# abhro/MonteCarloScattering.jl

Hardware: AMD Instinct MI355X
Metric: particle-scatter steps/sec + wall-time per iter, 10^6 particles, 1->8 MI355X (higher is better)
Workload: dtype f64

## Files before the change

montecarloscattering.jl_amd/csrc/mcs_transport.hip:

```cpp
#include "mcs_device.h"
#define MCS_DEVICE_FAST_SQRT 1
#include "../../include/mcs_math.h"
#include "../../include/mcs_math_f32.h"

#pragma clang fp contract(off)

#ifndef MCS_WAVES_PER_SIMD
#define MCS_WAVES_PER_SIMD 2
#endif
#ifndef MCS_REFILL_MIN
#define MCS_REFILL_MIN 12
#endif
#ifndef MCS_DEFER_K
#define MCS_DEFER_K 8
#endif
#ifndef MCS_PASSES_PER_ITER
#define MCS_PASSES_PER_ITER 6
#endif
#ifndef MCS_MERGE_POLL_MASK
#define MCS_MERGE_POLL_MASK 15u
#endif
#ifndef MCS_TAIL_CROSS
#define MCS_TAIL_CROSS 1
#endif
#ifdef MCS_INLINE_COLD
#define MCS_COLD __forceinline__
#else
#define MCS_COLD __noinline__
#endif

typedef const __attribute__((address_space(4))) KArgs CK;

namespace {

#define PI_ MCS_SC(3.141592653589793)
#define TWOPI_ MCS_SC(6.283185307179586)
#define HALFPI_ MCS_SC(1.5707963267948966)
#define SIN_UL MCS_SC(0x1.fffffffffffffp-1)
#define MP_ MCS_SC(MCS_MP)
#define CC_ MCS_SC(MCS_C)

__device__ __forceinline__ double rcp_refined(double b) {
  double r = __builtin_amdgcn_rcp(b);
// ... 1323 lines not shown
    else if (j == 6) off = a->L.energy_esc_feb + ion + (long long)a->P.n_ions * iter;
    if (v != 0.0) gadd_f64(&a->T[off], v);
  }
  for (int i = threadIdx.x; i < ng; i += blockDim.x) {
    const double v0 = S_fl[i], v1 = S_fl[MCS_MAXNE + i], v2 = S_fl[2 * MCS_MAXNE + i];
    if (v0 != 0.0) gadd_f64(&a->T[a->L.pxx_flux + i], v0);
    if (v1 != 0.0) gadd_f64(&a->T[a->L.pxz_flux + i], v1);
    if (v2 != 0.0) gadd_f64(&a->T[a->L.energy_flux + i], v2);
    const int c = S_nc[i];
    if (c) gadd_u64(&a->I[MCS_I_NUM_CROSSINGS + i], (unsigned long long)c);
  }
  for (int i = threadIdx.x; i < MCS_NA_C; i += blockDim.x) {
    const double w = S_wc[i];
    if (w != 0.0) gadd_f64(&a->T[a->L.weight_coupled + i + (long long)MCS_NA_C * (a->i_ion - 1)], w);
  }
  for (int i = threadIdx.x; i <= MCS_PSD_MAX; i += blockDim.x) {
    const long long o = i + (long long)(MCS_PSD_MAX + 1) * (a->i_ion - 1);
    const double e = S_eff[0][i], w = S_eff[1][i];
    if (e != 0.0) gadd_f64(&a->T[a->L.esc_energy_eff + o], e);
    if (w != 0.0) gadd_f64(&a->T[a->L.esc_num_eff + o], w);
  }
}

template <bool PLAIN, bool LOSSY = false, bool PLAIN_ETF = false, bool SLICED = false>
__device__ __forceinline__ void transport_body(const KArgs* __restrict__ ka) {
  CK* a = (CK*)ka;
  if (a->n_dev && *a->n_dev == 0) return;
  const int ne = a->P.n_grid + 2, ng = a->P.n_grid, ntc = a->tb.n_tcuts;
  block_prologue(a);
  __syncthreads();

  Hot h;
  h.m = vconst(a->m); h.x_grid_stop = vconst(a->P.x_grid_stop); h.xn_coarse = vconst(a->P.xn_per_coarse);
  h.u2 = sconst(a->P.u2); h.eta = sconst(a->P.eta_mfp); h.zzq = sconst(a->zzq); h.mc = sconst(a->mc);
  h.feb_down = sconst(a->P.feb_downstream); h.pcut = sconst(a->pcut); h.pmax_cutoff = sconst(a->pmax_cutoff);
  h.feb_up = sconst(a->P.feb_upstream); h.age_max = sconst(a->P.age_max); h.inj_frac = sconst(a->inj_frac);
  h.xn_fine = sconst(a->P.xn_per_fine); h.aa = sconst(a->aa);
  h.n_grid = sconsti(ng); h.i_grid_feb = sconsti(a->P.i_grid_feb); h.n_tcuts = sconsti(ntc); h.n_xspec = sconsti(a->tb.n_xspec);
  h.custom_epsB = a->P.use_custom_epsB != 0; h.etf = a->P.energy_transfer_frac > 0;
  h.dont_scatter = a->P.dont_scatter != 0; h.rad_losses = a->P.do_rad_losses != 0;
  h.do_tcuts = a->P.do_tcuts != 0; h.dont_DSA = a->P.dont_DSA != 0;
  {
    int ob = 0;
    for (int i = threadIdx.x; i < ne; i += blockDim.x) ob |= S_bsin[i] != 0.0;
    h.oblique = __builtin_amdgcn_readfirstlane(__syncthreads_or(ob)) != 0;
  }
  h.every_pass = h.custom_epsB || (h.rad_losses && h.aa < 1) || h.dont_scatter;
  h.odd_cfg = h.feb_down > 0 || h.dont_DSA || h.inj_frac < 1 || h.aa < 1 || h.n_xspec != 0;
  if (PLAIN) {
    h.custom_epsB = false; h.etf = PLAIN_ETF ? h.etf : false; h.dont_scatter = false; h.dont_DSA = false; h.oblique = false;
    h.every_pass = false; h.odd_cfg = false;
  }
  double l_bcmb = 0, l_pe_crit = 0, l_game_crit = 0;
  if (LOSSY) {
    h.every_pass = false; h.custom_epsB = false; h.dont_scatter = false; h.rad_losses = true;
    l_bcmb = sconst(a->P.B_CMBz); l_pe_crit = sconst(a->P.pe_crit); l_game_crit = sconst(a->P.game_crit);
  }

  mcsm::HotCoef kc;
  kc.S0 = vconst(MCS_SIN_0); kc.S1 = vconst(MCS_SIN_1); kc.S2 = vconst(MCS_SIN_2); kc.S3 = vconst(MCS_SIN_3);
  kc.S4 = vconst(MCS_SIN_4); kc.S5 = vconst(MCS_SIN_5);
  kc.C0 = vconst(MCS_COS_0); kc.C1 = vconst(MCS_COS_1); kc.C2 = vconst(MCS_COS_2); kc.C3 = vconst(MCS_COS_3);
  kc.C4 = vconst(MCS_COS_4); kc.C5 = vconst(MCS_COS_5);
  kc.A0 = vconst(MCS_ASIN_0); kc.A1 = vconst(MCS_ASIN_1); kc.A2 = vconst(MCS_ASIN_2); kc.A3 = vconst(MCS_ASIN_3);
  kc.A4 = vconst(MCS_ASIN_4); kc.A5 = vconst(MCS_ASIN_5); kc.A6 = vconst(MCS_ASIN_6); kc.A7 = vconst(MCS_ASIN_7);
  kc.A8 = vconst(MCS_ASIN_8); kc.A9 = vconst(MCS_ASIN_9); kc.A10 = vconst(MCS_ASIN_10); kc.A11 = vconst(MCS_ASIN_11);
  kc.A12 = vconst(MCS_ASIN_12);
  kc.R0 = vconst(MCS_TWO_OVER_PI); kc.R1 = vconst(MCS_PIO2_0); kc.R2 = vconst(MCS_PIO2_1); kc.R3 = vconst(MCS_PIO2_2);

  Pt p;
  Rng rng;
  p.weight = 0; p.ptot_pf = 1; p.pb_pf = 0; p.p_perp = 1; p.gam_pf = 1; p.x = 0; p.x_old = 0; p.phi = 0; p.prp = 0; p.acctime = 0;
  p.xn_per = 1; p.dphi = 0; p.gyro_denom = 0; p.gyro_rad = 0; p.gyro_rad_tot = 0; p.gyro_period = 0; p.t_step = 0;
  p.rp_val = 1; p.cm_val = 1; p.rg_val = 1; p.x_dt = 0; p.t_ev = 0; p.flags = 0; p.ovr_inc = 0; p.n_ovr = 0u;
  p.z_gsf = 1; p.z_bcos = 1; p.z_ux = 0; p.z_gef = 1; p.z_lo = 0; p.z_hi = 0; p.t_hi = 0; p.t_lo = 0; p.c_gef = 0; p.c_tev = 0;
  p.i_grid = 0; p.i_grid_old = 0; p.ig3 = 0; p.helix = 0; p.tcut = 1; p.n_retro = 0; p.downstream = false; p.inj = false;
  rng.init(0ull);
  int act = 0;
#define active (act != 0)
  bool exhausted = false;
  int evw = 0;
  double phi_prev = 0.0;
  long long k = -1;
  const unsigned lane = __lane_id();
  const unsigned long long n_resume = SLICED ? (unsigned long long)a->n_resume : 0ull;
  const long long fresh_lo = SLICED ? a->fresh_lo : 0ll;
  long long n_pop = a->n;
  if (a->n_dev) {
    const long long v = *a->n_dev;
    n_pop = (long long)(((unsigned long long)(unsigned)__builtin_amdgcn_readfirstlane((int)(v >> 32)) << 32) | (unsigned)__builtin_amdgcn_readfirstlane((int)v));
  }
  const unsigned long long n = n_resume + (unsigned long long)(n_pop - fresh_lo);
  const unsigned budget = SLICED ? (unsigned)__builtin_amdgcn_readfirstlane(a->budget_trips) : 0u;
  const int claim_max = SLICED ? __builtin_amdgcn_readfirstlane(a->claim_max) : 64;
  const unsigned long_draws = SLICED ? (unsigned)__builtin_amdgcn_readfirstlane((int)a->long_draws) : 0u;
  unsigned mtick_ex = 0;

  const unsigned wv = threadIdx.x >> 6;
  int mrole = 0;
  unsigned mtick = 0, mpoll_mask = ~0u;
  if (blockDim.x == 256u && a->tail_merge) {
    const unsigned s0 = S_msimd[0], s1 = S_msimd[1], s2 = S_msimd[2], s3 = S_msimd[3];
    const bool distinct = ((1u << s0) | (1u << s1) | (1u << s2) | (1u << s3)) == 15u;
    const unsigned slot = (unsigned)__builtin_amdgcn_s_getreg((3 << 11) | (0 << 6) | 4);
    if (__builtin_amdgcn_readfirstlane(distinct ? 1 : 0))
      mrole = __builtin_amdgcn_readfirstlane((int)(((S_msimd[wv] ^ slot) & 1u) == 0u ? 2 : 1));
  }
  auto pair_of = [&](unsigned& partner) -> unsigned {
    const unsigned mine = S_msimd[wv], want = mine ^ 1u;
    const unsigned pw = S_msimd[0] == want ? 0u : (S_msimd[1] == want ? 1u : (S_msimd[2] == want ? 2u : 3u));
    partner = (unsigned)__builtin_amdgcn_readfirstlane((int)pw);
    return (unsigned)__builtin_amdgcn_readfirstlane((int)(mine >> 1));
  };
#ifdef MCS_PROF
  const unsigned gw__ = (blockIdx.x * 4u + wv) & 8191u;
  if (lane == 0) { g_wave[gw__][0] = __builtin_amdgcn_s_memrealtime(); g_wave[gw__][1] = 0; }
  unsigned long long xp__ = 0, xr__ = 0, xl__ = 0, xf__ = 0;
#endif
  const bool waiting_on = __builtin_amdgcn_readfirstlane((int)(a->wait_full != 0 && blockDim.x == 256u)) != 0;
  const unsigned refill_min = claim_max < 64 ? (unsigned)(64 - claim_max + 1)
                                             : (unsigned)__builtin_amdgcn_readfirstlane(a->refill_min);
  unsigned refill_at = refill_min;
  unsigned ev_pending = 0;
  bool ring_on = false;
  unsigned rb = 0u - 256u;
  unsigned rrow = 0u;
  unsigned ringD = 1u;
  unsigned defer_k = h.every_pass ? 1u : (unsigned)__builtin_amdgcn_readfirstlane(a->defer_k);
  p.npush = 0;
  auto build_batch = [&](const unsigned long long am, const unsigned L) {
    const unsigned D = 64u / L;
    const unsigned M = 65536u / D + 1u;
    const unsigned rank = below(am);
    if (active) {
      S_evf[wv][3][128u + rank] = __hiloint2double((int)rng.k0, (int)rng.k1);
      S_evf[wv][4][128u + rank] = __hiloint2double((int)rng.n, 0);
      S_evf[wv][5][128u + rank] = 1 - p.cm_val;
    }
    const unsigned q = (lane * M) >> 16, jw = lane - q * D;
    const bool valid = q < L;
    const unsigned qq = valid ? q : 0u;
    const double w1 = S_evf[wv][3][128u + qq], w2 = S_evf[wv][4][128u + qq], womc = S_evf[wv][5][128u + qq];
    double eU1, es, ec, ecd, esd, essd;
    scatter_draws((uint32_t)__double2hiint(w1), (uint32_t)__double2loint(w1), ((uint32_t)__double2hiint(w2) >> 1) + jw, kc, eU1, es, ec);
    scatter_cone(eU1, es, womc, ecd, esd, essd);
    if (valid) {
      S_evf[wv][0][128u + lane] = ecd; S_evf[wv][1][128u + lane] = esd; S_evf[wv][2][128u + lane] = ec; S_evf[wv][6][128u + lane] = essd;
    }
    if (active) { rb = rng.n; rrow = rank * D; }
    ringD = D;
  };
  constexpr bool TAIL_LOOP = !LOSSY;
  const unsigned tail_loop_L = TAIL_LOOP ? (unsigned)__builtin_amdgcn_readfirstlane(a->tail_loop) : 0u;
  bool done = false;
  while (!done) {
    ev_pending += (unsigned)(__popcll(__builtin_amdgcn_ballot_w64(p.npush > 0)) + __popcll(__builtin_amdgcn_ballot_w64(p.npush > 1)));
    p.npush = 0;
    const unsigned long long act_mask = __builtin_amdgcn_ballot_w64(active);
    const int n_idle = 64 - __popcll(act_mask);
    unsigned Lh = 64u - (unsigned)n_idle;
    const bool waitl = (p.flags & F_WAIT) != 0;
    const unsigned n_wait = (unsigned)__popcll(__builtin_amdgcn_ballot_w64(waitl));
    ++mtick;
    if (MCS_UNLIKELY(((ev_pending >= 64u) | ((unsigned)n_idle + n_wait >= refill_at) | ((mtick & mpoll_mask) == 0u)) != 0)) {
      if (ev_pending >= 64u) { drain_events(a, wv, lane, false); ev_pending &= 63u; PROF_ADD(3, 1); }
      if (n_wait > 0u && (exhausted || (unsigned)n_idle + n_wait >= refill_min)) {
        if (waitl) p.flags = (p.flags & ~F_WAIT) | F_NOPARK;
        PROF_ADD(36, 1); PROF_ADD(37, n_wait);
      }
      const unsigned long long idle = ~__builtin_amdgcn_ballot_w64(active);
      if ((unsigned)n_idle + n_wait >= refill_min && !exhausted && idle != 0ull) {
        const int nfree = __popcll(idle);
        int nidle = nfree < claim_max - (64 - nfree) ? nfree : claim_max - (64 - nfree);
        nidle = nidle > 0 ? nidle : 0;
        const int leader = __ffsll((long long)idle) - 1;
        unsigned long long base = 0;
        if ((int)lane == leader) base = atomicAdd(a->work_counter, (unsigned long long)nidle);
        base = __shfl(base, leader);
        if (__builtin_amdgcn_readfirstlane(base >= n ? 1 : 0)) {
          exhausted = true;
          defer_k = 1u;
          ring_on = !LOSSY && __builtin_amdgcn_readfirstlane(a->tail_ring) != 0;
          mtick_ex = mtick;
          if (mrole != 0 || budget != 0u) mpoll_mask = MCS_MERGE_POLL_MASK;
#ifdef MCS_PROF_TAIL
          if (lane == 0) S_ttgate[wv] = 1u;
#endif
#ifdef MCS_PROF
          if (lane == 0 && g_wave[gw__][1] == 0) { g_wave[gw__][1] = __builtin_amdgcn_s_memrealtime(); g_wave[gw__][3] = (unsigned long long)__popcll(act_mask); }
#endif
        } else if (!active) {
          const int rank = (int)below(idle);
          const unsigned long long idx = base + (unsigned long long)rank;
          if (rank < nidle && idx >= n_resume && idx < n) {
            k = fresh_lo + (long long)(idx - n_resume);
            load_particle(a, h, k, p, rng);
            act = -1; evw = 0; rb = 0u - 256u;
            __builtin_amdgcn_s_waitcnt(0x0F70);
          }
        }
        if (SLICED && !exhausted && __builtin_amdgcn_readfirstlane(base < n_resume ? 1 : 0)) {
          drain_events(a, wv, lane, true); ev_pending = 0u;
          const unsigned long long left = n_resume - base;
          const unsigned cnt_r = (unsigned)(left < (unsigned long long)nidle ? left : (unsigned long long)nidle);
          const unsigned rank = below(idle);
          double* const box = &S_evf[wv][0][0];
          for (unsigned b0 = 0; b0 < cnt_r; b0 += MCS_MB_SLOTS) {
            const unsigned cb = cnt_r - b0 < MCS_MB_SLOTS ? cnt_r - b0 : MCS_MB_SLOTS;
            const double* src = a->strag_in + (base + b0) * MCS_STRAG_WORDS;
            for (unsigned i = lane; i < MCS_MB_WORDS * MCS_MB_SLOTS; i += 64u) {
              const unsigned j = i / MCS_MB_SLOTS, r = i % MCS_MB_SLOTS;
              if (r < cb) box[i] = src[r * MCS_STRAG_WORDS + j];
            }
            __builtin_amdgcn_fence(__ATOMIC_RELEASE, "wavefront"); __builtin_amdgcn_wave_barrier(); __builtin_amdgcn_fence(__ATOMIC_ACQUIRE, "wavefront");
            if (!active && rank >= b0 && rank < b0 + cb) {
              mb_load(wv, rank - b0, p, rng, k, evw, phi_prev);
              refresh_thr<LOSSY>(h, p);
              act = -1; rb = rng.n - 256u;
            }
            __builtin_amdgcn_fence(__ATOMIC_RELEASE, "wavefront"); __builtin_amdgcn_wave_barrier(); __builtin_amdgcn_fence(__ATOMIC_ACQUIRE, "wavefront");
          }
        }
        PROF_ADD(5, 1); PROF_ADD(6, nidle);
      }
      auto take_donation = [&](unsigned mpair, unsigned mpartner) {
        __builtin_amdgcn_fence(__ATOMIC_ACQUIRE, "workgroup");
        const unsigned cntm = (unsigned)__builtin_amdgcn_readfirstlane((int)S_mcount[mpair]);
        const unsigned long long idle_now = ~__builtin_amdgcn_ballot_w64(active);
        const unsigned r = below(idle_now);
        if (!active && r < cntm) {
          mb_load(mpartner, r, p, rng, k, evw, phi_prev);
          refresh_thr<LOSSY>(h, p);
          rb = rng.n - 256u;
          act = -1;
        }
        mrole = 0; mpoll_mask = budget != 0u ? MCS_MERGE_POLL_MASK : ~0u;
      };
      const bool closing = SLICED && budget != 0u && exhausted &&
                           (long_draws != 0u ? __builtin_amdgcn_ballot_w64(active && rng.n < long_draws) == 0ull : mtick - mtick_ex >= budget);
      if (mrole != 0 && exhausted) {
        unsigned mpartner;
        const unsigned mpair = pair_of(mpartner);
        const int nlive = __popcll(__builtin_amdgcn_ballot_w64(active));
        if (mrole == 2) {
          unsigned st = 0u;
          if (lane == 0) {
            S_mlive[wv] = (unsigned)nlive;
            st = (nlive == 0 || closing) ? atomicCAS(&S_mstate[mpair], 0u, 2u) : __hip_atomic_load(&S_mstate[mpair], __ATOMIC_RELAXED, __HIP_MEMORY_SCOPE_WORKGROUP);
          }
          st = (unsigned)__builtin_amdgcn_readfirstlane((int)st);
          if (st == 1u) {
            take_donation(mpair, mpartner);
            if (lane == 0) S_mstate[mpair] = 2u;
          } else if (st == 2u || nlive == 0 || closing) { mrole = 0; mpoll_mask = budget != 0u ? MCS_MERGE_POLL_MASK : ~0u; }
        } else {
          const int room = 64 - (int)__builtin_amdgcn_readfirstlane((int)S_mlive[mpartner]);
          if (nlive == 0 || closing) {
            if (lane == 0) (void)atomicCAS(&S_mstate[mpair], 0u, 2u);
            mrole = 0; mpoll_mask = budget != 0u ? MCS_MERGE_POLL_MASK : ~0u;
          } else if (nlive <= MCS_MB_SLOTS && nlive <= room) {
            drain_events(a, wv, lane, true); ev_pending = 0u;
            if (active) mb_store(wv, below(__builtin_amdgcn_ballot_w64(active)), p, rng, k, evw, phi_prev);
            rb = rng.n - 256u;
// ... 15 lines not shown
          const int nlive = __popcll(am_x);
          const int leader = __ffsll((long long)am_x) - 1;
          unsigned long long base = 0;
          if ((int)lane == leader) base = atomicAdd(a->strag_count, (unsigned long long)nlive);
          base = __shfl(base, leader);
          drain_events(a, wv, lane, true); ev_pending = 0u;
          const unsigned rank = below(am_x);
          double* const box = &S_evf[wv][0][0];
          for (unsigned b0 = 0; b0 < (unsigned)nlive; b0 += MCS_MB_SLOTS) {
            const unsigned cb = (unsigned)nlive - b0 < MCS_MB_SLOTS ? (unsigned)nlive - b0 : MCS_MB_SLOTS;
            if (active && rank >= b0 && rank < b0 + cb) mb_store(wv, rank - b0, p, rng, k, evw, phi_prev);
            __builtin_amdgcn_fence(__ATOMIC_RELEASE, "wavefront"); __builtin_amdgcn_wave_barrier(); __builtin_amdgcn_fence(__ATOMIC_ACQUIRE, "wavefront");
            double* dst = a->strag_out + (base + b0) * MCS_STRAG_WORDS;
            for (unsigned i = lane; i < MCS_MB_WORDS * MCS_MB_SLOTS; i += 64u) {
              const unsigned j = i / MCS_MB_SLOTS, r = i % MCS_MB_SLOTS;
              if (r < cb) dst[r * MCS_STRAG_WORDS + j] = box[i];
            }
            __builtin_amdgcn_fence(__ATOMIC_RELEASE, "wavefront"); __builtin_amdgcn_wave_barrier(); __builtin_amdgcn_fence(__ATOMIC_ACQUIRE, "wavefront");
          }
          act = 0; p.flags = 0; p.helix = 0; evw = 0;
        }
        mrole = 0;
      }
      if (exhausted) refill_at = 64u;
      const unsigned long long am_hk = __builtin_amdgcn_ballot_w64(active);
      Lh = (unsigned)__popcll(am_hk);
      done = (am_hk == 0ull) & exhausted;
    }
    {
      [[maybe_unused]] const int na__ = __popcll(__builtin_amdgcn_ballot_w64(active));
      PROF_ADD(0, 1); PROF_ADD(8, na__);
#ifdef MCS_PROF
      if (exhausted) { xp__ += 1; xl__ += (unsigned long long)na__; }
#endif
    }
    double t_clock = p.t_step;
    const int wi = (((evw & 3) | p.flags) | (h.every_pass ? 1 : 0)) & act;
    const bool waits = (p.flags & F_WAIT) != 0;
    const bool want = (wi != 0) & !waits;
    PROF_LANES(13, want);
#ifdef MCS_PROF_TAIL
    const bool rare_any__ = PROF_GATE && __builtin_amdgcn_ballot_w64(want) != 0ull;
    unsigned long long tt0__ = 0;
    if (rare_any__) tt0__ = __builtin_amdgcn_s_memtime();
#endif
    bool waits_now = false;
    bool loss_done = false;
    const unsigned long long m_want = __builtin_amdgcn_ballot_w64(want);
    const unsigned long long m_urgent = __builtin_amdgcn_ballot_w64(want & ((wi & F_NOPARK) != 0));
    const bool enter = (m_urgent != 0ull) | ((unsigned)__popcll(m_want) >= defer_k);
    if (MCS_UNLIKELY(want & enter)) {
      PROF_ADD(12, 1);
#ifdef MCS_PROF_TAIL
#define TT_MARK(slot) do { const unsigned long long tn__ = __builtin_amdgcn_s_memtime(); if (PROF_GATE && (threadIdx.x & 63u) == (unsigned)(__ffsll((long long)__ballot(1)) - 1)) atomicAdd(&S_prof[slot], tn__ - tm__); tm__ = __builtin_amdgcn_s_memtime(); } while (0)
      unsigned long long tm__ = __builtin_amdgcn_s_memtime();
#else
#define TT_MARK(slot) do { } while (0)
#endif
      const double cm_in = p.cm_val;
      const bool moved = (evw & 4) != 0, thr = (evw & 2) != 0;
      bool ev = (evw & 1) != 0, ev_x = false;
      bool up_due = false, xn_due = false, feb_due = false;
      if (__builtin_amdgcn_ballot_w64(thr) != 0ull) {
        const bool fwd = p.x > p.x_old;
        const bool same_zone = (fwd & (p.z_hi > p.x)) | (!fwd & (p.z_lo <= p.x));
        const bool ev_up = ((p.x >= h.x_grid_stop) & ((p.x_old < h.x_grid_stop) | ((p.x_old < p.prp) & (p.x >= p.prp)))) | (p.x > p.x_dt);
        const bool ev_xn = !LOSSY & ((p.x > p.gyro_rad_tot) != (p.xn_per == h.xn_coarse));
        ev_x = thr & !same_zone;
        up_due = thr & ev_up; xn_due = thr & ev_xn;
        feb_due = thr & (p.i_grid <= h.i_grid_feb) & p.inj & (p.x < h.feb_up);
        ev = ev | up_due | xn_due | feb_due;
      }
      [[maybe_unused]] const bool unusual = (p.flags != 0) | (p.helix >= MCS_HELIX_CAP) | h.every_pass;
      const bool post_pending = moved && (ev || ev_x || (p.flags & F_INJCHK) != 0);
      int end = -1;
      bool t_due = false, age_out = false;
      if (__builtin_amdgcn_ballot_w64(ev) != 0ull) {
        t_due = ev & p.downstream & (p.acctime >= p.t_ev);
        age_out = (h.age_max > 0) & (p.acctime > h.age_max);
      }
      const bool etf_due = h.etf & ev_x & !(p.inj | (p.downstream & (p.x < 0))) & (p.x_old <= 0);
      bool full = (p.flags & ~F_CM) != 0 || p.helix >= MCS_HELIX_CAP || h.every_pass || etf_due || h.custom_epsB ||
                  (ev && (h.odd_cfg || up_due || age_out || feb_due));
      TT_MARK(32);
      if (!full && ev_x) full = !plain_crossing(a, h, p, ev_pending);
      TT_MARK(33);
      if (waiting_on && !exhausted) {
        waits_now = full & moved & ((p.flags & F_NOPARK) == 0);
        p.flags = waits_now ? (p.flags | F_WAIT) : p.flags;
        full = full & !waits_now;
      }
      if (__builtin_amdgcn_ballot_w64(full || (!waits_now && ((p.flags & F_CM) != 0 || t_due || xn_due))) != 0ull) {
      if (!full && !waits_now) {
        if (p.flags & F_CM) {
          refresh_scatter(a, p, h.aa, h.aa * MP_ * CC_, h.eta);
          p.flags = 0;
        }
        if (t_due) {
          if (h.do_tcuts && !(p.tcut > h.n_tcuts) && p.acctime >= tcut_next_of(a, h, p.tcut)) {
            tcut_track(a, p.tcut, p.weight, p.ptot_pf);
            p.tcut += 1;
          }
          refresh_time(a, h, p);
        }
        if (xn_due) {
          p.xn_per = p.x > p.gyro_rad_tot ? h.xn_coarse : h.xn_fine;
          p.flags |= F_CM;
          refresh_move(a, h, p);
        }
      }
// ... 41 lines not shown
          a->sv.xn_per[k] = p.xn_per;
          a->sv.prp_x_cm[k] = p.x < p.prp ? p.prp : p.x * 1.1;
          a->sv.acctime_sec[k] = p.acctime; a->sv.phi_rad[k] = p.phi;
          a->sv.meta[k] = mcs_pack_meta(p.i_grid, p.tcut, p.downstream, p.inj);
          cnt(a, MCS_IC_COUNT);
        } else {
          a->l_save[k] = SLICED ? (uint8_t)(2u | ((long_draws != 0u && rng.n >= long_draws) ? 4u : 0u)) : (uint8_t)2;
          if (p.npush < 2) {
            push_record(p, p.ig3, -1, (1u << 28) | ((uint32_t)end << 25));
          } else {
            particle_finish(a, end, p.pb_pf, p.p_perp, p.gam_pf, p.phi, p.weight, p.ig3);
          }
        }
        cnt(a, MCS_IC_REASON0 + end);
        if (a->f_reason) {
          a->f_reason[k] = end; a->f_helix[k] = p.helix; a->f_retro[k] = p.n_retro; a->f_ptot[k] = p.ptot_pf; a->f_x[k] = p.x;
        }
        act = 0;
        p.flags = 0; p.helix = 0;
        TT_MARK(19);
      }
      }
      if (!waits_now) refresh_thr<LOSSY>(h, p);
      if (MCS_UNLIKELY(ring_on)) rb = (p.cm_val != cm_in) ? rng.n - 256u : rb;
    }
    const bool frozen = want & !enter;
#ifdef MCS_PROF_TAIL
    if (rare_any__) { const unsigned long long dt__ = __builtin_amdgcn_s_memtime() - tt0__; if (lane == 0) { atomicAdd(&S_prof[30], dt__); atomicAdd(&S_prof[31], 1ull); } }
#endif
    bool run = !frozen & ((p.flags & F_WAIT) == 0);
    const bool may_go_on = (p.flags == 0) & !h.every_pass;
    bool stopped = false;
    bool tail_fast = false;
    unsigned long long am_t = 0ull;
    if constexpr (TAIL_LOOP) {
      if (MCS_UNLIKELY(ring_on)) {
        am_t = __builtin_amdgcn_ballot_w64(active);
        tail_fast = (Lh <= tail_loop_L) & (am_t != 0ull) & (__builtin_amdgcn_ballot_w64(active & !run) == 0ull);
      }
    }
    if (MCS_UNLIKELY(tail_fast)) {
      unsigned jj = (rng.n - rb) >> 1;
      if (__builtin_amdgcn_ballot_w64(active && jj >= ringD) != 0ull) {
        build_batch(am_t, (unsigned)__popcll(am_t));
        jj = 0u;
      }
      unsigned e = (rrow + jj) & 63u;
      const unsigned long long m_halt = __builtin_amdgcn_ballot_w64(!may_go_on);
      TailK K;
      K.halfpi = sconst(MCS_PIO2_DD_0); K.pio2_lo = sconst(MCS_PIO2_DD_1); K.twopi = sconst(MCS_TWOPI_DD_0); K.twopi_lo = sconst(MCS_TWOPI_DD_1);
      K.inv_twopi = sconst(MCS_INV_TWOPI); K.sin_ul = sconst(0x1.fffffffffffffp-1); K.dmin = sconst(2.2250738585072014e-308);
#pragma nounroll
      for (;;) {
        PROF_LANES(9, active); PROF_ADD(7, 1);
        p.helix += 1;
        if (!h.dont_scatter) {
          rng.n += 2u;
          const double cos_d = S_evf[wv][0][128u + e], sin_d = S_evf[wv][1][128u + e], c_ps = S_evf[wv][2][128u + e], ssd = S_evf[wv][6][128u + e];
          scattering_rest_k(p, kc, K, cos_d, sin_d, c_ps, ssd);
        }
        p.acctime = p.acctime + t_clock * p.c_gef;
        p.n_ovr += (unsigned)p.ovr_inc;
        const bool ev_time = p.acctime >= p.c_tev;
        bool x1;
        const bool e1 = move_and_detect_thr(a, h, p, phi_prev, x1, true, &K) | ev_time | (p.helix >= MCS_HELIX_CAP);
        evw = (e1 ? 5 : 4) | (x1 ? 2 : 0);
        e = (e + 1u) & 63u; jj += 1u;
        t_clock = p.t_step;
        const unsigned long long m_stop = __builtin_amdgcn_ballot_w64(e1 | x1 | (jj >= ringD)) | m_halt;
        if ((m_stop & am_t) != 0ull) break;
      }
      if (MCS_TAIL_CROSS) {
        ev_pending += (unsigned)(__popcll(__builtin_amdgcn_ballot_w64(p.npush > 0)) + __popcll(__builtin_amdgcn_ballot_w64(p.npush > 1)));
        p.npush = 0;
        if (ev_pending < 64u) {
          if (active & ((evw & 3) == 2) & (p.flags == 0) & !(h.etf | h.odd_cfg | h.custom_epsB | h.every_pass)) {
            const bool fwd = p.x > p.x_old;
            const bool same_zone = (fwd & (p.z_hi > p.x)) | (!fwd & (p.z_lo <= p.x));
            const bool ev_up = ((p.x >= h.x_grid_stop) & ((p.x_old < h.x_grid_stop) | ((p.x_old < p.prp) & (p.x >= p.prp)))) | (p.x > p.x_dt);
            const bool ev_xn = (p.x > p.gyro_rad_tot) != (p.xn_per == h.xn_coarse);
            const bool feb_due = (p.i_grid <= h.i_grid_feb) & p.inj & (p.x < h.feb_up);
            if (!(ev_up | ev_xn | feb_due)) {
              const bool handled = same_zone ? true : plain_crossing(a, h, p, ev_pending);
              if (handled) { refresh_thr<false>(h, p); evw = 4; }
            }
          }
        }
      }
    } else
#pragma unroll
    for (int rep = 0; rep < MCS_PASSES_PER_ITER; ++rep) {
      if (rep > 0) {
        run = run & may_go_on & !stopped;
        t_clock = p.t_step;
      }
      stopped = false;
      bool got = false;
      unsigned ridx = 0u;
      if (MCS_UNLIKELY(ring_on)) {
        const unsigned long long am = __builtin_amdgcn_ballot_w64(active);
        const unsigned L = (unsigned)__popcll(am);
        if ((L >= 1u) & (Lh <= 32u)) {
          unsigned jj = (rng.n - rb) >> 1;
          if (__builtin_amdgcn_ballot_w64(active && jj >= ringD) != 0ull) {
            build_batch(am, L);
            jj = 0u;
          }
          ridx = (rrow + jj) & 63u;
          got = true;
        } else {
          rb = rng.n - 256u;
        }
      }
      PROF_LANES(9, run & active); PROF_ADD(7, 1);
      if constexpr (LOSSY) {
        if (run && !(rep == 0 && loss_done)) {
          const double bmag = S_bt[p.ig3];
          const double ptot_old = p.ptot_pf;
          const double B_CMB_loc = l_bcmb * p.z_gef;
          double pn;
          {
            const double dlnp = MCS_RAD_LOSS_FAC * (bmag * bmag + B_CMB_loc * B_CMB_loc) * ptot_old * t_clock;
// ... 33 lines not shown
          rng.n = jd + 2u;
          if (got) { cos_d = S_evf[wv][0][128u + ridx]; sin_d = S_evf[wv][1][128u + ridx]; c_ps = S_evf[wv][2][128u + ridx]; ssd = S_evf[wv][6][128u + ridx]; }
          else {
            double U1, s_ps;
            scatter_draws(rng.k0, rng.k1, jd >> 1, kc, U1, s_ps, c_ps);
            scatter_cone(U1, s_ps, 1 - p.cm_val, cos_d, sin_d, ssd);
          }
          scattering_rest(p, kc, cos_d, sin_d, c_ps, ssd);
        }
        {
          p.acctime = p.acctime + t_clock * p.c_gef;
          p.n_ovr += (unsigned)p.ovr_inc;
          const bool ev_time = p.acctime >= p.c_tev;
          bool x1;
          const bool e1 = move_and_detect_thr(a, h, p, phi_prev, x1, !LOSSY) | ev_time | (p.helix >= MCS_HELIX_CAP);
          evw = (e1 ? 5 : 4) | (x1 ? 2 : 0);
          stopped = e1 | x1;
        }
      }
    }
  }

#ifdef MCS_PROF
  if (lane == 0) { g_wave[gw__][2] = __builtin_amdgcn_s_memrealtime(); g_wave[gw__][4] = xp__; g_wave[gw__][6] = xl__;
    g_wave[gw__][5] = (unsigned long long)__builtin_amdgcn_s_getreg((31 << 11) | (0 << 6) | 4);
    g_wave[gw__][7] = (unsigned long long)__builtin_amdgcn_s_getreg((31 << 11) | (0 << 6) | 20); }
#endif
  drain_events(a, wv, lane, true);
  __syncthreads();
#ifdef MCS_PROF
  if (threadIdx.x < MCS_NPROF && S_prof[threadIdx.x]) atomicAdd(&g_prof[threadIdx.x], S_prof[threadIdx.x]);
#endif
  block_flush(a);
}

#undef active

extern "C" __global__ void __launch_bounds__(256, MCS_WAVES_PER_SIMD) mcs_k_transport(const KArgs* __restrict__ ka) {
  transport_body<false>(ka);
}
extern "C" __global__ void __launch_bounds__(256, MCS_WAVES_PER_SIMD) mcs_k_transport_plain(const KArgs* __restrict__ ka) {
  transport_body<true>(ka);
}
extern "C" __global__ void __launch_bounds__(256, MCS_WAVES_PER_SIMD) mcs_k_transport_lossy(const KArgs* __restrict__ ka) {
  transport_body<false, true>(ka);
}
extern "C" __global__ void __launch_bounds__(256, MCS_WAVES_PER_SIMD) mcs_k_transport_plain_etf(const KArgs* __restrict__ ka) {
  transport_body<true, false, true>(ka);
}
extern "C" __global__ void __launch_bounds__(256, MCS_WAVES_PER_SIMD) mcs_k_transport_sliced(const KArgs* __restrict__ ka) {
  transport_body<false, false, false, true>(ka);
}
extern "C" __global__ void __launch_bounds__(256, MCS_WAVES_PER_SIMD) mcs_k_transport_plain_sliced(const KArgs* __restrict__ ka) {
  transport_body<true, false, false, true>(ka);
}
extern "C" __global__ void __launch_bounds__(256, MCS_WAVES_PER_SIMD) mcs_k_transport_lossy_sliced(const KArgs* __restrict__ ka) {
  transport_body<false, true, false, true>(ka);
}
extern "C" __global__ void __launch_bounds__(256, MCS_WAVES_PER_SIMD) mcs_k_transport_plain_etf_sliced(const KArgs* __restrict__ ka) {
// ... 28 lines not shown
```

Measured before the change: 44.78 billion.

## Split transport loop into separately compiled main and tail phases

The single transport loop is split into two template instances: a main phase that claims and refills work, and a noinline tail phase entered once the work counter is exhausted. State is handed over through a LaneState struct. Each phase compiles only its own logic, so the main loop sheds the ring, merge and donation code and should need fewer registers. The tail phase gains an occupancy-scaled defer rule (MCS_TAIL_DEFER_DIV) and a fast-loop continuation (MCS_TAIL_BACK) that keeps iterating without going back to housekeeping, at the cost of a spill/copy of lane state and a noinline call boundary.

```diff
diff --git a/montecarloscattering.jl_amd/csrc/mcs_transport.hip b/montecarloscattering.jl_amd/csrc/mcs_transport.hip
--- a/montecarloscattering.jl_amd/csrc/mcs_transport.hip
+++ b/montecarloscattering.jl_amd/csrc/mcs_transport.hip
@@ -19,6 +19,12 @@
 #endif
 #ifndef MCS_MERGE_POLL_MASK
 #define MCS_MERGE_POLL_MASK 15u
+#endif
+#ifndef MCS_TAIL_DEFER_DIV
+#define MCS_TAIL_DEFER_DIV 8u
+#endif
+#ifndef MCS_TAIL_BACK
+#define MCS_TAIL_BACK 1
 #endif
 #ifndef MCS_TAIL_CROSS
 #define MCS_TAIL_CROSS 1
@@ -1388,42 +1394,48 @@
   }
 }
 
-template <bool PLAIN, bool LOSSY = false, bool PLAIN_ETF = false, bool SLICED = false>
-__device__ __forceinline__ void transport_body(const KArgs* __restrict__ ka) {
-  CK* a = (CK*)ka;
-  if (a->n_dev && *a->n_dev == 0) return;
-  const int ne = a->P.n_grid + 2, ng = a->P.n_grid, ntc = a->tb.n_tcuts;
-  block_prologue(a);
-  __syncthreads();
-
-  Hot h;
+struct LaneState {
+  Pt p;
+  Rng rng;
+  long long k;
+  double phi_prev;
+  int act, evw;
+  unsigned ev_pending;
+  int oblique;
+};
+
+template <bool RFL>
+__device__ __forceinline__ int uni_i32(int x) { return RFL ? __builtin_amdgcn_readfirstlane(x) : x; }
+template <bool RFL>
+__device__ __forceinline__ double uni_f64(double x) {
+  return RFL ? __hiloint2double(__builtin_amdgcn_readfirstlane(__double2hiint(x)), __builtin_amdgcn_readfirstlane(__double2loint(x))) : x;
+}
+template <bool PLAIN, bool LOSSY, bool PLAIN_ETF, bool RFL>
+__device__ __forceinline__ void hot_setup(CK* a, const bool oblique, Hot& h, double& l_bcmb, double& l_pe_crit, double& l_game_crit) {
+  const int ng = a->P.n_grid, ntc = a->tb.n_tcuts;
   h.m = vconst(a->m); h.x_grid_stop = vconst(a->P.x_grid_stop); h.xn_coarse = vconst(a->P.xn_per_coarse);
-  h.u2 = sconst(a->P.u2); h.eta = sconst(a->P.eta_mfp); h.zzq = sconst(a->zzq); h.mc = sconst(a->mc);
-  h.feb_down = sconst(a->P.feb_downstream); h.pcut = sconst(a->pcut); h.pmax_cutoff = sconst(a->pmax_cutoff);
-  h.feb_up = sconst(a->P.feb_upstream); h.age_max = sconst(a->P.age_max); h.inj_frac = sconst(a->inj_frac);
-  h.xn_fine = sconst(a->P.xn_per_fine); h.aa = sconst(a->aa);
-  h.n_grid = sconsti(ng); h.i_grid_feb = sconsti(a->P.i_grid_feb); h.n_tcuts = sconsti(ntc); h.n_xspec = sconsti(a->tb.n_xspec);
+  h.u2 = sconst(uni_f64<RFL>(a->P.u2)); h.eta = sconst(uni_f64<RFL>(a->P.eta_mfp)); h.zzq = sconst(uni_f64<RFL>(a->zzq)); h.mc = sconst(uni_f64<RFL>(a->mc));
+  h.feb_down = sconst(uni_f64<RFL>(a->P.feb_downstream)); h.pcut = sconst(uni_f64<RFL>(a->pcut)); h.pmax_cutoff = sconst(uni_f64<RFL>(a->pmax_cutoff));
+  h.feb_up = sconst(uni_f64<RFL>(a->P.feb_upstream)); h.age_max = sconst(uni_f64<RFL>(a->P.age_max)); h.inj_frac = sconst(uni_f64<RFL>(a->inj_frac));
+  h.xn_fine = sconst(uni_f64<RFL>(a->P.xn_per_fine)); h.aa = sconst(uni_f64<RFL>(a->aa));
+  h.n_grid = sconsti(uni_i32<RFL>(ng)); h.i_grid_feb = sconsti(uni_i32<RFL>(a->P.i_grid_feb)); h.n_tcuts = sconsti(uni_i32<RFL>(ntc)); h.n_xspec = sconsti(uni_i32<RFL>(a->tb.n_xspec));
   h.custom_epsB = a->P.use_custom_epsB != 0; h.etf = a->P.energy_transfer_frac > 0;
   h.dont_scatter = a->P.dont_scatter != 0; h.rad_losses = a->P.do_rad_losses != 0;
   h.do_tcuts = a->P.do_tcuts != 0; h.dont_DSA = a->P.dont_DSA != 0;
-  {
-    int ob = 0;
-    for (int i = threadIdx.x; i < ne; i += blockDim.x) ob |= S_bsin[i] != 0.0;
-    h.oblique = __builtin_amdgcn_readfirstlane(__syncthreads_or(ob)) != 0;
-  }
+  h.oblique = oblique;
   h.every_pass = h.custom_epsB || (h.rad_losses && h.aa < 1) || h.dont_scatter;
   h.odd_cfg = h.feb_down > 0 || h.dont_DSA || h.inj_frac < 1 || h.aa < 1 || h.n_xspec != 0;
   if (PLAIN) {
     h.custom_epsB = false; h.etf = PLAIN_ETF ? h.etf : false; h.dont_scatter = false; h.dont_DSA = false; h.oblique = false;
     h.every_pass = false; h.odd_cfg = false;
   }
-  double l_bcmb = 0, l_pe_crit = 0, l_game_crit = 0;
+  l_bcmb = 0; l_pe_crit = 0; l_game_crit = 0;
   if (LOSSY) {
     h.every_pass = false; h.custom_epsB = false; h.dont_scatter = false; h.rad_losses = true;
-    l_bcmb = sconst(a->P.B_CMBz); l_pe_crit = sconst(a->P.pe_crit); l_game_crit = sconst(a->P.game_crit);
-  }
-
-  mcsm::HotCoef kc;
+    l_bcmb = sconst(uni_f64<RFL>(a->P.B_CMBz)); l_pe_crit = sconst(uni_f64<RFL>(a->P.pe_crit)); l_game_crit = sconst(uni_f64<RFL>(a->P.game_crit));
+  }
+}
+__device__ __forceinline__ void hotcoef_setup(mcsm::HotCoef& kc) {
   kc.S0 = vconst(MCS_SIN_0); kc.S1 = vconst(MCS_SIN_1); kc.S2 = vconst(MCS_SIN_2); kc.S3 = vconst(MCS_SIN_3);
   kc.S4 = vconst(MCS_SIN_4); kc.S5 = vconst(MCS_SIN_5);
   kc.C0 = vconst(MCS_COS_0); kc.C1 = vconst(MCS_COS_1); kc.C2 = vconst(MCS_COS_2); kc.C3 = vconst(MCS_COS_3);
@@ -1433,46 +1445,44 @@
   kc.A8 = vconst(MCS_ASIN_8); kc.A9 = vconst(MCS_ASIN_9); kc.A10 = vconst(MCS_ASIN_10); kc.A11 = vconst(MCS_ASIN_11);
   kc.A12 = vconst(MCS_ASIN_12);
   kc.R0 = vconst(MCS_TWO_OVER_PI); kc.R1 = vconst(MCS_PIO2_0); kc.R2 = vconst(MCS_PIO2_1); kc.R3 = vconst(MCS_PIO2_2);
-
-  Pt p;
-  Rng rng;
-  p.weight = 0; p.ptot_pf = 1; p.pb_pf = 0; p.p_perp = 1; p.gam_pf = 1; p.x = 0; p.x_old = 0; p.phi = 0; p.prp = 0; p.acctime = 0;
-  p.xn_per = 1; p.dphi = 0; p.gyro_denom = 0; p.gyro_rad = 0; p.gyro_rad_tot = 0; p.gyro_period = 0; p.t_step = 0;
-  p.rp_val = 1; p.cm_val = 1; p.rg_val = 1; p.x_dt = 0; p.t_ev = 0; p.flags = 0; p.ovr_inc = 0; p.n_ovr = 0u;
-  p.z_gsf = 1; p.z_bcos = 1; p.z_ux = 0; p.z_gef = 1; p.z_lo = 0; p.z_hi = 0; p.t_hi = 0; p.t_lo = 0; p.c_gef = 0; p.c_tev = 0;
-  p.i_grid = 0; p.i_grid_old = 0; p.ig3 = 0; p.helix = 0; p.tcut = 1; p.n_retro = 0; p.downstream = false; p.inj = false;
-  rng.init(0ull);
-  int act = 0;
+}
+
+template <bool PLAIN, bool LOSSY, bool PLAIN_ETF, bool SLICED, bool TAIL>
+__device__ __forceinline__ void transport_phase(CK* a, const Hot& h, const mcsm::HotCoef& kc, const double l_bcmb, const double l_pe_crit,
+                                                const double l_game_crit, Pt& p, Rng& rng, long long& k, double& phi_prev, int& act,
+                                                int& evw, unsigned& ev_pending) {
 #define active (act != 0)
-  bool exhausted = false;
-  int evw = 0;
-  double phi_prev = 0.0;
-  long long k = -1;
+  [[maybe_unused]] constexpr bool exhausted = TAIL;
   const unsigned lane = __lane_id();
-  const unsigned long long n_resume = SLICED ? (unsigned long long)a->n_resume : 0ull;
-  const long long fresh_lo = SLICED ? a->fresh_lo : 0ll;
-  long long n_pop = a->n;
-  if (a->n_dev) {
-    const long long v = *a->n_dev;
-    n_pop = (long long)(((unsigned long long)(unsigned)__builtin_amdgcn_readfirstlane((int)(v >> 32)) << 32) | (unsigned)__builtin_amdgcn_readfirstlane((int)v));
-  }
-  const unsigned long long n = n_resume + (unsigned long long)(n_pop - fresh_lo);
-  const unsigned budget = SLICED ? (unsigned)__builtin_amdgcn_readfirstlane(a->budget_trips) : 0u;
-  const int claim_max = SLICED ? __builtin_amdgcn_readfirstlane(a->claim_max) : 64;
+  [[maybe_unused]] const unsigned long long n_resume = SLICED ? (unsigned long long)a->n_resume : 0ull;
+  [[maybe_unused]] const long long fresh_lo = SLICED ? a->fresh_lo : 0ll;
+  [[maybe_unused]] unsigned long long n = 0ull;
+  if constexpr (!TAIL) {
+    long long n_pop = a->n;
+    if (a->n_dev) {
+      const long long v = *a->n_dev;
+      n_pop = (long long)(((unsigned long long)(unsigned)__builtin_amdgcn_readfirstlane((int)(v >> 32)) << 32) | (unsigned)__builtin_amdgcn_readfirstlane((int)v));
+    }
+    n = n_resume + (unsigned long long)(n_pop - fresh_lo);
+  }
+  [[maybe_unused]] const unsigned budget = (SLICED && TAIL) ? (unsigned)__builtin_amdgcn_readfirstlane(a->budget_trips) : 0u;
+  [[maybe_unused]] const int claim_max = SLICED ? __builtin_amdgcn_readfirstlane(a->claim_max) : 64;
   const unsigned long_draws = SLICED ? (unsigned)__builtin_amdgcn_readfirstlane((int)a->long_draws) : 0u;
-  unsigned mtick_ex = 0;
+  [[maybe_unused]] unsigned mtick_ex = 0;
 
   const unsigned wv = threadIdx.x >> 6;
-  int mrole = 0;
-  unsigned mtick = 0, mpoll_mask = ~0u;
-  if (blockDim.x == 256u && a->tail_merge) {
-    const unsigned s0 = S_msimd[0], s1 = S_msimd[1], s2 = S_msimd[2], s3 = S_msimd[3];
-    const bool distinct = ((1u << s0) | (1u << s1) | (1u << s2) | (1u << s3)) == 15u;
-    const unsigned slot = (unsigned)__builtin_amdgcn_s_getreg((3 << 11) | (0 << 6) | 4);
-    if (__builtin_amdgcn_readfirstlane(distinct ? 1 : 0))
-      mrole = __builtin_amdgcn_readfirstlane((int)(((S_msimd[wv] ^ slot) & 1u) == 0u ? 2 : 1));
-  }
-  auto pair_of = [&](unsigned& partner) -> unsigned {
+  [[maybe_unused]] int mrole = 0;
+  [[maybe_unused]] unsigned mtick = 0, mpoll_mask = 0u;
+  if constexpr (TAIL) {
+    if (blockDim.x == 256u && a->tail_merge) {
+      const unsigned s0 = S_msimd[0], s1 = S_msimd[1], s2 = S_msimd[2], s3 = S_msimd[3];
+      const bool distinct = ((1u << s0) | (1u << s1) | (1u << s2) | (1u << s3)) == 15u;
+      const unsigned slot = (unsigned)__builtin_amdgcn_s_getreg((3 << 11) | (0 << 6) | 4);
+      if (__builtin_amdgcn_readfirstlane(distinct ? 1 : 0))
+        mrole = __builtin_amdgcn_readfirstlane((int)(((S_msimd[wv] ^ slot) & 1u) == 0u ? 2 : 1));
+    }
+  }
+  [[maybe_unused]] auto pair_of = [&](unsigned& partner) -> unsigned {
     const unsigned mine = S_msimd[wv], want = mine ^ 1u;
     const unsigned pw = S_msimd[0] == want ? 0u : (S_msimd[1] == want ? 1u : (S_msimd[2] == want ? 2u : 3u));
     partner = (unsigned)__builtin_amdgcn_readfirstlane((int)pw);
@@ -1480,21 +1490,20 @@
   };
 #ifdef MCS_PROF
   const unsigned gw__ = (blockIdx.x * 4u + wv) & 8191u;
-  if (lane == 0) { g_wave[gw__][0] = __builtin_amdgcn_s_memrealtime(); g_wave[gw__][1] = 0; }
+  if (!TAIL && lane == 0) { g_wave[gw__][0] = __builtin_amdgcn_s_memrealtime(); g_wave[gw__][1] = 0; }
   unsigned long long xp__ = 0, xr__ = 0, xl__ = 0, xf__ = 0;
 #endif
-  const bool waiting_on = __builtin_amdgcn_readfirstlane((int)(a->wait_full != 0 && blockDim.x == 256u)) != 0;
-  const unsigned refill_min = claim_max < 64 ? (unsigned)(64 - claim_max + 1)
+  [[maybe_unused]] const bool waiting_on = !TAIL && __builtin_amdgcn_readfirstlane((int)(a->wait_full != 0 && blockDim.x == 256u)) != 0;
+  [[maybe_unused]] const unsigned refill_min = TAIL ? 64u : claim_max < 64 ? (unsigned)(64 - claim_max + 1)
                                              : (unsigned)__builtin_amdgcn_readfirstlane(a->refill_min);
-  unsigned refill_at = refill_min;
-  unsigned ev_pending = 0;
-  bool ring_on = false;
-  unsigned rb = 0u - 256u;
-  unsigned rrow = 0u;
-  unsigned ringD = 1u;
-  unsigned defer_k = h.every_pass ? 1u : (unsigned)__builtin_amdgcn_readfirstlane(a->defer_k);
-  p.npush = 0;
-  auto build_batch = [&](const unsigned long long am, const unsigned L) {
+  const unsigned refill_at = refill_min;
+  [[maybe_unused]] bool ring_on = false;
+  if constexpr (TAIL && !LOSSY) ring_on = __builtin_amdgcn_readfirstlane(a->tail_ring) != 0;
+  [[maybe_unused]] unsigned rb = rng.n - 256u;
+  [[maybe_unused]] unsigned rrow = 0u;
+  [[maybe_unused]] unsigned ringD = 1u;
+  [[maybe_unused]] const unsigned defer_k = (TAIL || h.every_pass) ? 1u : (unsigned)__builtin_amdgcn_readfirstlane(a->defer_k);
+  [[maybe_unused]] auto build_batch = [&](const unsigned long long am, const unsigned L) {
     const unsigned D = 64u / L;
     const unsigned M = 65536u / D + 1u;
     const unsigned rank = below(am);
@@ -1516,7 +1525,7 @@
     if (active) { rb = rng.n; rrow = rank * D; }
     ringD = D;
   };
-  constexpr bool TAIL_LOOP = !LOSSY;
+  constexpr bool TAIL_LOOP = TAIL && !LOSSY;
   const unsigned tail_loop_L = TAIL_LOOP ? (unsigned)__builtin_amdgcn_readfirstlane(a->tail_loop) : 0u;
   bool done = false;
   while (!done) {
@@ -1524,18 +1533,19 @@
     p.npush = 0;
     const unsigned long long act_mask = __builtin_amdgcn_ballot_w64(active);
     const int n_idle = 64 - __popcll(act_mask);
-    unsigned Lh = 64u - (unsigned)n_idle;
-    const bool waitl = (p.flags & F_WAIT) != 0;
-    const unsigned n_wait = (unsigned)__popcll(__builtin_amdgcn_ballot_w64(waitl));
-    ++mtick;
-    if (MCS_UNLIKELY(((ev_pending >= 64u) | ((unsigned)n_idle + n_wait >= refill_at) | ((mtick & mpoll_mask) == 0u)) != 0)) {
+    [[maybe_unused]] unsigned Lh = 64u - (unsigned)n_idle;
+    const bool waitl = !TAIL && (p.flags & F_WAIT) != 0;
+    const unsigned n_wait = TAIL ? 0u : (unsigned)__popcll(__builtin_amdgcn_ballot_w64(waitl));
+    if constexpr (TAIL) ++mtick;
+    if (MCS_UNLIKELY(((ev_pending >= 64u) | ((unsigned)n_idle + n_wait >= refill_at) | (TAIL && (mtick & mpoll_mask) == 0u)) != 0)) {
       if (ev_pending >= 64u) { drain_events(a, wv, lane, false); ev_pending &= 63u; PROF_ADD(3, 1); }
-      if (n_wait > 0u && (exhausted || (unsigned)n_idle + n_wait >= refill_min)) {
+      if constexpr (!TAIL) {
+      if (n_wait > 0u && (unsigned)n_idle + n_wait >= refill_min) {
         if (waitl) p.flags = (p.flags & ~F_WAIT) | F_NOPARK;
         PROF_ADD(36, 1); PROF_ADD(37, n_wait);
       }
       const unsigned long long idle = ~__builtin_amdgcn_ballot_w64(active);
-      if ((unsigned)n_idle + n_wait >= refill_min && !exhausted && idle != 0ull) {
+      if ((unsigned)n_idle + n_wait >= refill_min && idle != 0ull) {
         const int nfree = __popcll(idle);
         int nidle = nfree < claim_max - (64 - nfree) ? nfree : claim_max - (64 - nfree);
         nidle = nidle > 0 ? nidle : 0;
@@ -1544,28 +1554,24 @@
         if ((int)lane == leader) base = atomicAdd(a->work_counter, (unsigned long long)nidle);
         base = __shfl(base, leader);
         if (__builtin_amdgcn_readfirstlane(base >= n ? 1 : 0)) {
-          exhausted = true;
-          defer_k = 1u;
-          ring_on = !LOSSY && __builtin_amdgcn_readfirstlane(a->tail_ring) != 0;
-          mtick_ex = mtick;
-          if (mrole != 0 || budget != 0u) mpoll_mask = MCS_MERGE_POLL_MASK;
 #ifdef MCS_PROF_TAIL
           if (lane == 0) S_ttgate[wv] = 1u;
 #endif
 #ifdef MCS_PROF
           if (lane == 0 && g_wave[gw__][1] == 0) { g_wave[gw__][1] = __builtin_amdgcn_s_memrealtime(); g_wave[gw__][3] = (unsigned long long)__popcll(act_mask); }
 #endif
+          done = true;
         } else if (!active) {
           const int rank = (int)below(idle);
           const unsigned long long idx = base + (unsigned long long)rank;
           if (rank < nidle && idx >= n_resume && idx < n) {
             k = fresh_lo + (long long)(idx - n_resume);
             load_particle(a, h, k, p, rng);
-            act = -1; evw = 0; rb = 0u - 256u;
+            act = -1; evw = 0;
             __builtin_amdgcn_s_waitcnt(0x0F70);
           }
         }
-        if (SLICED && !exhausted && __builtin_amdgcn_readfirstlane(base < n_resume ? 1 : 0)) {
+        if (SLICED && !done && __builtin_amdgcn_readfirstlane(base < n_resume ? 1 : 0)) {
           drain_events(a, wv, lane, true); ev_pending = 0u;
           const unsigned long long left = n_resume - base;
           const unsigned cnt_r = (unsigned)(left < (unsigned long long)nidle ? left : (unsigned long long)nidle);
@@ -1582,12 +1588,17 @@
             if (!active && rank >= b0 && rank < b0 + cb) {
               mb_load(wv, rank - b0, p, rng, k, evw, phi_prev);
               refresh_thr<LOSSY>(h, p);
-              act = -1; rb = rng.n - 256u;
+              act = -1;
             }
             __builtin_amdgcn_fence(__ATOMIC_RELEASE, "wavefront"); __builtin_amdgcn_wave_barrier(); __builtin_amdgcn_fence(__ATOMIC_ACQUIRE, "wavefront");
           }
         }
         PROF_ADD(5, 1); PROF_ADD(6, nidle);
+      }
+      } else {
+      if (mtick == 1u) {
+        mtick_ex = mtick;
+        mpoll_mask = (mrole != 0 || budget != 0u) ? MCS_MERGE_POLL_MASK : ~0u;
       }
       auto take_donation = [&](unsigned mpair, unsigned mpartner) {
         __builtin_amdgcn_fence(__ATOMIC_ACQUIRE, "workgroup");
@@ -1602,9 +1613,9 @@
         }
         mrole = 0; mpoll_mask = budget != 0u ? MCS_MERGE_POLL_MASK : ~0u;
       };
-      const bool closing = SLICED && budget != 0u && exhausted &&
+      const bool closing = SLICED && budget != 0u &&
                            (long_draws != 0u ? __builtin_amdgcn_ballot_w64(active && rng.n < long_draws) == 0ull : mtick - mtick_ex >= budget);
-      if (mrole != 0 && exhausted) {
+      if (mrole != 0) {
         unsigned mpartner;
         const unsigned mpair = pair_of(mpartner);
         const int nlive = __popcll(__builtin_amdgcn_ballot_w64(active));
@@ -1666,10 +1677,10 @@
         }
         mrole = 0;
       }
-      if (exhausted) refill_at = 64u;
       const unsigned long long am_hk = __builtin_amdgcn_ballot_w64(active);
       Lh = (unsigned)__popcll(am_hk);
-      done = (am_hk == 0ull) & exhausted;
+      done = am_hk == 0ull;
+      }
     }
     {
       [[maybe_unused]] const int na__ = __popcll(__builtin_amdgcn_ballot_w64(active));
@@ -1680,7 +1691,7 @@
     }
     double t_clock = p.t_step;
     const int wi = (((evw & 3) | p.flags) | (h.every_pass ? 1 : 0)) & act;
-    const bool waits = (p.flags & F_WAIT) != 0;
+    const bool waits = !TAIL && (p.flags & F_WAIT) != 0;
     const bool want = (wi != 0) & !waits;
     PROF_LANES(13, want);
 #ifdef MCS_PROF_TAIL
@@ -1692,7 +1703,9 @@
     bool loss_done = false;
     const unsigned long long m_want = __builtin_amdgcn_ballot_w64(want);
     const unsigned long long m_urgent = __builtin_amdgcn_ballot_w64(want & ((wi & F_NOPARK) != 0));
-    const bool enter = (m_urgent != 0ull) | ((unsigned)__popcll(m_want) >= defer_k);
+    bool enter;
+    if constexpr (TAIL) enter = MCS_TAIL_DEFER_DIV == 0 || ((m_urgent != 0ull) | (Lh <= (TAIL_LOOP ? tail_loop_L : 12u)) | ((unsigned)__popcll(m_want) * MCS_TAIL_DEFER_DIV >= Lh));
+    else enter = (m_urgent != 0ull) | ((unsigned)__popcll(m_want) >= defer_k);
     if (MCS_UNLIKELY(want & enter)) {
       PROF_ADD(12, 1);
 #ifdef MCS_PROF_TAIL
@@ -1701,7 +1714,7 @@
 #else
 #define TT_MARK(slot) do { } while (0)
 #endif
-      const double cm_in = p.cm_val;
+      [[maybe_unused]] const double cm_in = p.cm_val;
       const bool moved = (evw & 4) != 0, thr = (evw & 2) != 0;
       bool ev = (evw & 1) != 0, ev_x = false;
       bool up_due = false, xn_due = false, feb_due = false;
@@ -1729,7 +1742,7 @@
       TT_MARK(32);
       if (!full && ev_x) full = !plain_crossing(a, h, p, ev_pending);
       TT_MARK(33);
-      if (waiting_on && !exhausted) {
+      if (!TAIL && waiting_on && !done) {
         waits_now = full & moved & ((p.flags & F_NOPARK) == 0);
         p.flags = waits_now ? (p.flags | F_WAIT) : p.flags;
         full = full & !waits_now;
@@ -1817,24 +1830,24 @@
       }
       }
       if (!waits_now) refresh_thr<LOSSY>(h, p);
-      if (MCS_UNLIKELY(ring_on)) rb = (p.cm_val != cm_in) ? rng.n - 256u : rb;
+      if constexpr (TAIL) { if (MCS_UNLIKELY(ring_on)) rb = (p.cm_val != cm_in) ? rng.n - 256u : rb; }
     }
     const bool frozen = want & !enter;
 #ifdef MCS_PROF_TAIL
     if (rare_any__) { const unsigned long long dt__ = __builtin_amdgcn_s_memtime() - tt0__; if (lane == 0) { atomicAdd(&S_prof[30], dt__); atomicAdd(&S_prof[31], 1ull); } }
 #endif
-    bool run = !frozen & ((p.flags & F_WAIT) == 0);
+    bool run = !frozen & (TAIL || (p.flags & F_WAIT) == 0);
     const bool may_go_on = (p.flags == 0) & !h.every_pass;
     bool stopped = false;
     bool tail_fast = false;
-    unsigned long long am_t = 0ull;
+    [[maybe_unused]] unsigned long long am_t = 0ull;
     if constexpr (TAIL_LOOP) {
-      if (MCS_UNLIKELY(ring_on)) {
+      if (ring_on) {
         am_t = __builtin_amdgcn_ballot_w64(active);
         tail_fast = (Lh <= tail_loop_L) & (am_t != 0ull) & (__builtin_amdgcn_ballot_w64(active & !run) == 0ull);
       }
     }
-    if (MCS_UNLIKELY(tail_fast)) {
+    if constexpr (TAIL_LOOP) if (tail_fast) {
       unsigned jj = (rng.n - rb) >> 1;
       if (__builtin_amdgcn_ballot_w64(active && jj >= ringD) != 0ull) {
         build_batch(am_t, (unsigned)__popcll(am_t));
@@ -1845,6 +1858,7 @@
       TailK K;
       K.halfpi = sconst(MCS_PIO2_DD_0); K.pio2_lo = sconst(MCS_PIO2_DD_1); K.twopi = sconst(MCS_TWOPI_DD_0); K.twopi_lo = sconst(MCS_TWOPI_DD_1);
       K.inv_twopi = sconst(MCS_INV_TWOPI); K.sin_ul = sconst(0x1.fffffffffffffp-1); K.dmin = sconst(2.2250738585072014e-308);
+      for (;;) {
 #pragma nounroll
       for (;;) {
         PROF_LANES(9, active); PROF_ADD(7, 1);
@@ -1880,9 +1894,18 @@
               if (handled) { refresh_thr<false>(h, p); evw = 4; }
             }
           }
+          if (MCS_TAIL_BACK && (m_halt & am_t) == 0ull &&
+              __builtin_amdgcn_ballot_w64(active & (((evw & 3) != 0) | (p.flags != 0) | (jj >= ringD))) == 0ull &&
+              ((mtick + 1u) & mpoll_mask) != 0u) {
+            ++mtick;
+            continue;
+          }
         }
       }
-    } else
+      break;
+      }
+    }
+    if (!tail_fast)
 #pragma unroll
     for (int rep = 0; rep < MCS_PASSES_PER_ITER; ++rep) {
       if (rep > 0) {
@@ -1892,7 +1915,7 @@
       stopped = false;
       bool got = false;
       unsigned ridx = 0u;
-      if (MCS_UNLIKELY(ring_on)) {
+      if (TAIL && ring_on) {
         const unsigned long long am = __builtin_amdgcn_ballot_w64(active);
         const unsigned L = (unsigned)__popcll(am);
         if ((L >= 1u) & (Lh <= 32u)) {
@@ -1972,11 +1995,39 @@
   }
 
 #ifdef MCS_PROF
-  if (lane == 0) { g_wave[gw__][2] = __builtin_amdgcn_s_memrealtime(); g_wave[gw__][4] = xp__; g_wave[gw__][6] = xl__;
-    g_wave[gw__][5] = (unsigned long long)__builtin_amdgcn_s_getreg((31 << 11) | (0 << 6) | 4);
-    g_wave[gw__][7] = (unsigned long long)__builtin_amdgcn_s_getreg((31 << 11) | (0 << 6) | 20); }
-#endif
-  drain_events(a, wv, lane, true);
+  if (TAIL && lane == 0) { g_wave[gw__][4] = xp__; g_wave[gw__][6] = xl__; }
+#endif
+#undef active
+}
+
+template <bool PLAIN, bool LOSSY, bool PLAIN_ETF, bool SLICED>
+__device__ __noinline__ void transport_tail(CK* a, const LaneState* ls) {
+  Hot h;
+  double l_bcmb, l_pe_crit, l_game_crit;
+  hot_setup<PLAIN, LOSSY, PLAIN_ETF, true>(a, __builtin_amdgcn_readfirstlane(ls->oblique) != 0, h, l_bcmb, l_pe_crit, l_game_crit);
+  mcsm::HotCoef kc;
+  hotcoef_setup(kc);
+  Pt p = ls->p;
+  Rng rng = ls->rng;
+  long long k = ls->k;
+  double phi_prev = ls->phi_prev;
+  int act = ls->act, evw = ls->evw;
+  unsigned ev_pending = (unsigned)__builtin_amdgcn_readfirstlane((int)ls->ev_pending);
+  transport_phase<PLAIN, LOSSY, PLAIN_ETF, SLICED, true>(a, h, kc, l_bcmb, l_pe_crit, l_game_crit, p, rng, k, phi_prev, act, evw, ev_pending);
+}
+
+template <bool PLAIN, bool LOSSY, bool PLAIN_ETF, bool SLICED>
+__device__ __noinline__ void transport_epilogue(CK* a) {
+#ifdef MCS_PROF
+  {
+    const unsigned lane = __lane_id();
+    const unsigned gw__ = (blockIdx.x * 4u + (threadIdx.x >> 6)) & 8191u;
+    if (lane == 0) { g_wave[gw__][2] = __builtin_amdgcn_s_memrealtime();
+      g_wave[gw__][5] = (unsigned long long)__builtin_amdgcn_s_getreg((31 << 11) | (0 << 6) | 4);
+      g_wave[gw__][7] = (unsigned long long)__builtin_amdgcn_s_getreg((31 << 11) | (0 << 6) | 20); }
+  }
+#endif
+  drain_events(a, threadIdx.x >> 6, __lane_id(), true);
   __syncthreads();
 #ifdef MCS_PROF
   if (threadIdx.x < MCS_NPROF && S_prof[threadIdx.x]) atomicAdd(&g_prof[threadIdx.x], S_prof[threadIdx.x]);
@@ -1984,7 +2035,49 @@
   block_flush(a);
 }
 
-#undef active
+template <bool PLAIN, bool LOSSY = false, bool PLAIN_ETF = false, bool SLICED = false>
+__device__ __forceinline__ void transport_body(const KArgs* __restrict__ ka) {
+  CK* a = (CK*)ka;
+  if (a->n_dev && *a->n_dev == 0) return;
+  const int ne = a->P.n_grid + 2;
+  block_prologue(a);
+  __syncthreads();
+
+  bool oblique;
+  {
+    int ob = 0;
+    for (int i = threadIdx.x; i < ne; i += blockDim.x) ob |= S_bsin[i] != 0.0;
+    oblique = __builtin_amdgcn_readfirstlane(__syncthreads_or(ob)) != 0;
+  }
+  Hot h;
+  double l_bcmb, l_pe_crit, l_game_crit;
+  hot_setup<PLAIN, LOSSY, PLAIN_ETF, false>(a, oblique, h, l_bcmb, l_pe_crit, l_game_crit);
+  mcsm::HotCoef kc;
+  hotcoef_setup(kc);
+
+  Pt p;
+  Rng rng;
+  p.weight = 0; p.ptot_pf = 1; p.pb_pf = 0; p.p_perp = 1; p.gam_pf = 1; p.x = 0; p.x_old = 0; p.phi = 0; p.prp = 0; p.acctime = 0;
+  p.xn_per = 1; p.dphi = 0; p.gyro_denom = 0; p.gyro_rad = 0; p.gyro_rad_tot = 0; p.gyro_period = 0; p.t_step = 0;
+  p.rp_val = 1; p.cm_val = 1; p.rg_val = 1; p.x_dt = 0; p.t_ev = 0; p.flags = 0; p.ovr_inc = 0; p.n_ovr = 0u;
+  p.z_gsf = 1; p.z_bcos = 1; p.z_ux = 0; p.z_gef = 1; p.z_lo = 0; p.z_hi = 0; p.t_hi = 0; p.t_lo = 0; p.c_gef = 0; p.c_tev = 0;
+  p.i_grid = 0; p.i_grid_old = 0; p.ig3 = 0; p.helix = 0; p.tcut = 1; p.n_retro = 0; p.downstream = false; p.inj = false;
+  p.npush = 0;
+  rng.init(0ull);
+  int act = 0;
+  int evw = 0;
+  double phi_prev = 0.0;
+  long long k = -1;
+  unsigned ev_pending = 0;
+  transport_phase<PLAIN, LOSSY, PLAIN_ETF, SLICED, false>(a, h, kc, l_bcmb, l_pe_crit, l_game_crit, p, rng, k, phi_prev, act, evw, ev_pending);
+  {
+    LaneState ls;
+    ls.p = p; ls.rng = rng; ls.k = k; ls.phi_prev = phi_prev; ls.act = act; ls.evw = evw; ls.ev_pending = ev_pending;
+    ls.oblique = oblique ? 1 : 0;
+    transport_tail<PLAIN, LOSSY, PLAIN_ETF, SLICED>(a, &ls);
+  }
+  transport_epilogue<PLAIN, LOSSY, PLAIN_ETF, SLICED>(a);
+}
 
 extern "C" __global__ void __launch_bounds__(256, MCS_WAVES_PER_SIMD) mcs_k_transport(const KArgs* __restrict__ ka) {
   transport_body<false>(ka);
```

Measured after the change: 44.65 billion. No clear change (-0.3%).
